# RomanBresson/KAGNN

Hardware: AMD Instinct MI355X
Metric: edges/sec KAN-GIN fwd+bwd, hidden=64 grid=5, 1M-node synthetic; HBM % peak (higher is better)
Workload: dtype f32 (fp16 hi/lo split operands, fp32 accumulate)

## Files before the change

### kagnn_amd/csrc/kan_split_bwd.hip

```cpp
#include <type_traits>
#include "split_common.h"

namespace kagnn {

int kan_dw_reduce(const float* slab, long NS, long per_slab, float* gcat, hipStream_t st);

int kan_dw_unpack(const float* gcat, int in, int out, int C, long inP, long outP, const float* sw,
                  const float* sc, float* g_bw, float* g_sw, float* g_sc, hipStream_t st);


bool kan_split_dx_ok(int in, int out, int G, int K) { return K >= 0 && K <= 4 && G + K <= 16; }
static inline int vshift(int C) { return C > 8 ? 1 : 0; }

static size_t dx_blk_bytes(int inv , int ob) {
    return kHdrBytes + (size_t)cdiv(inv, 16) * kCTmax * dx_q2(ob) * 2 * 1024;
}
bool kan_dx_w2_ok(int in, int out, int C, int K) { return K == 3 && C > 8 && C <= 16 && out <= kOutBlk; }
static int dx_inv(int in, int out, int C, int K) { return kan_dx_w2_ok(in, out, C, K) ? 32 * cdiv(in, 16) : (in << vshift(C)); }

size_t kan_split_pack_dx_bytes(int in, int out, int C, int K) {
    return (size_t)cdiv(out, kOutBlk) * dx_blk_bytes(dx_inv(in, out, C, K), min(out, kOutBlk));
}

__global__ void split_pack_dx_kernel(const float* __restrict__ bw, const float* __restrict__ sw,
                                     const float* __restrict__ sc, int in, int out, int C, int Q2,
                                     unsigned char* __restrict__ pack, int self_scale, int w2) {
    unsigned* hdr = reinterpret_cast<unsigned*>(pack);
    __shared__ float s_m[17];
    const float wmax = self_scale == 2 ? header_absmax(pack) : self_scale ? block_absmax_w(bw, sw, sc, in, out, C, s_m) : __uint_as_float(hdr[2]);
    const int e = scale_exp_from_max(wmax);
    const float wscale = ldexpf(1.0f, -e);
    if (blockIdx.x == 0 && threadIdx.x == 0) {
        reinterpret_cast<float*>(pack)[0] = ldexpf(1.0f, e - 10);
        reinterpret_cast<int*>(pack)[1] = e;
    }
    pack_dx_items(bw, sw, sc, in, out, C, Q2, pack, wscale, blockIdx.x * (long)blockDim.x + threadIdx.x, (long)gridDim.x * blockDim.x, w2);
}

int kan_split_pack_dx_noscale(const float* bw, const float* sw, const float* sc, int in, int out, int C, int K,
                              void* pack_dx, hipStream_t st) {
    const int w2 = kan_dx_w2_ok(in, out, C, K) ? 1 : 0;
    const int inv = dx_inv(in, out, C, K);
    const size_t stride = dx_blk_bytes(inv, min(out, kOutBlk));
    for (int b = 0; b * kOutBlk < out; ++b) {
        const int ob = min(kOutBlk, out - b * kOutBlk), Q2 = dx_q2(ob);
        const long o0 = (long)b * kOutBlk;
        const long items = (long)cdiv(inv, 16) * kCTmax * Q2 * 64;
        const bool two = (long)in * ob * C >= kAbsmaxTwoLaunchMin;
        unsigned char* pd = static_cast<unsigned char*>(pack_dx) + b * stride;
        if (two) { int rc = launch_absmax_partials(bw ? bw + o0 * in : nullptr, sw + o0 * in * C, sc ? sc + o0 * in : nullptr, in, ob, C, pd, st); if (rc) return rc; }
        split_pack_dx_kernel<<<(int)min((items + 1023) / 1024, two ? 256L : 64L), 1024, 0, st>>>(
            bw ? bw + o0 * in : nullptr, sw + o0 * in * C, sc ? sc + o0 * in : nullptr, in, ob, C, Q2, pd, two ? 2 : 1, w2);
        KAGNN_LAUNCH_CHECK();
    }
    return KAGNN_OK;
}

template <int K>
__device__ __forceinline__ float barrel_dot(const float (&d)[8], int m, const float (&dN)[K + 1]) {
    const int a = m >> 2, b = m & 3;
    float U[K + 4];
#pragma unroll
    for (int j = 0; j < K + 4; ++j) {
        float v = 0.0f;
#pragma unroll
        for (int aa = 0; aa < 4; ++aa) {
            const int c = 4 * aa + j - K;
            if (c >= 0 && c < 8) v = (a == aa) ? d[c] : v;
        }
        U[j] = v;
    }
    float s = 0.0f;
#pragma unroll
    for (int r = 0; r <= K; ++r) {
        float e = U[r];
#pragma unroll
        for (int bb = 1; bb < 4; ++bb) e = (b == bb) ? U[r + bb] : e;
        s = fmaf(e, dN[r], s);
    }
    return s;
}


template <int K, int Q2, bool GEN, int PP, bool GX16 = false, bool BNB = false, bool XAFF = false, bool XST = false, bool HALF = false>
__global__ __launch_bounds__(512) void kan_split_dx_kernel(
    const float* __restrict__ x, long ldx, const float* __restrict__ gy, long ldgy, long N, int in,
    int out, int C, const float* __restrict__ knots_g, int nknots,
    const unsigned char* __restrict__ pack, int resident, float* __restrict__ gx, long ldgx,
    RbfArgs rb, int sh_arg , int acc_arg,
    int ft_per_block , BnBack bnb) {
    static_assert(!BNB || (K == 3 && !GEN && PP == 0 && !GX16), "the fused normalisation backward serves the lean cubic instantiation");
    static_assert(!XAFF || (K == 3 && !GEN && !GX16 && !BNB), "the input affine serves the lean cubic instantiation (the read-out of the node models)");
    static_assert(!XST || XAFF, "the column statistics ride in the read-out instantiation");
    static_assert(!HALF || (K == 3 && !GEN), "single-product mode: the lean cubic instantiation");
    const int sh = GEN ? sh_arg : 0;
    const bool ACC = GEN && acc_arg;
    extern __shared__ __attribute__((aligned(16))) unsigned char smem[];
    float* s_knots = reinterpret_cast<float*>(smem);
    unsigned char* s_w = smem + kLdsHdr;
    const int tid = threadIdx.x, wave = tid >> 6, lane = tid & 63;
    if (K > 0 && tid < nknots) s_knots[tid] = knots_g[tid];
    unsigned* s_btbl = reinterpret_cast<unsigned*>(smem + 256);
    constexpr unsigned gxes = GX16 ? 2u : 4u;
    if (K == 3) build_barrel_table(s_btbl, tid);
    const int inv = in << sh, FT = cdiv(inv, 16);
    constexpr int FT_BYTES = kCTmax * Q2 * 2 * 1024;
    const int e_w = reinterpret_cast<const int*>(pack)[1];
    const unsigned char* gw = pack + kHdrBytes;
    const unsigned lds_w = (unsigned)(size_t)((__attribute__((address_space(3))) unsigned char*)s_w);
    auto stage = [&](int ft0, int nft) {
        const unsigned char* src = gw + (size_t)ft0 * FT_BYTES;
        const int nblk = nft * (FT_BYTES / 1024);
        if constexpr (HALF) {
            for (int blk = 2 * wave; blk < nblk; blk += 16)
                lds_dma_1k(src + (size_t)blk * 1024 + lane * 16, __builtin_amdgcn_readfirstlane(lds_w + blk * 1024));
        } else
        for (int blk = wave; blk < nblk; blk += 8)
            lds_dma_1k(src + (size_t)blk * 1024 + lane * 16, __builtin_amdgcn_readfirstlane(lds_w + blk * 1024));
        lds_dma_wait();
    };
    const int ft_begin = blockIdx.y * ft_per_block, ft_end = min(FT, ft_begin + ft_per_block);
    if (resident) stage(ft_begin, ft_end - ft_begin);
    __syncthreads();
    const bool pingpong = (PP == 2) && resident;
    SplineGeom geom{}; FastGeom fgeo{};
    const int li = lane & 15, kg = lane >> 4;
    const int win = li & sh;
    float ca[8] = {};
    if constexpr (K == 0) {
        float c0[8], c1[8];
        rbf_centers(rb, c0, 0); rbf_centers(rb, c1, sh);
#pragma unroll
        for (int g = 0; g < 8; ++g) ca[g] = win ? c1[g] : c0[g];
    }
    if constexpr (K > 0) { geom = geom_from_knots(s_knots, nknots); fgeo = fast_geom(s_knots, nknots); }
    const bool ln_on = (K == 0) && rb.ln_w != nullptr;
    const bool al4 = ((ldgy & 3) == 0) && ((reinterpret_cast<uintptr_t>(gy) & 15) == 0);
    const unsigned ldx4 = (unsigned)ldx * 4u, ldgy4 = (unsigned)ldgy * 4u, ldgx4 = (unsigned)ldgx * gxes;
    const unsigned gy_ro = (unsigned)(wave * 32 + li) * ldgy4;
    const unsigned x_rb = (unsigned)(wave * 32 + 4 * kg) * ldx4;
    const unsigned gx_rb = (unsigned)(wave * 32 + 4 * kg) * ldgx4;
    const unsigned gz_rb = (unsigned)(wave * 32 + 4 * kg) * (unsigned)in * 4u;

    auto load_gy = [&](long tile, float (&raw)[2][Q2][8]) {
        const GBuf gyb = gbuf_at(gy, N, ldgy, out, tile * 256);
#pragma unroll
        for (int rt = 0; rt < 2; ++rt) {
            const unsigned ro = gy_ro + kg * 32;
            const unsigned so = (unsigned)(16 * rt) * ldgy4;
#pragma unroll
            for (int q = 0; q < Q2; ++q) {
                if (al4 && 32 * Q2 == out) {
                    gld4_s(gyb, ro, so + 128 * q, raw[rt][q]);
                    gld4_s(gyb, ro, so + 128 * q + 16, raw[rt][q] + 4);
                } else if (al4 && (out & 7) == 0) {
                    const unsigned rq = gy_ro + (unsigned)min(32 * q + 8 * kg, out - 8) * 4u;
                    gld4_s(gyb, rq, so, raw[rt][q]);
                    gld4_s(gyb, rq, so + 16, raw[rt][q] + 4);
                } else {
                    const int o0 = 32 * q + 8 * kg;
#pragma unroll
                    for (int j = 0; j < 8; ++j) raw[rt][q][j] = gld_s(gyb, gy_ro + min(o0 + j, out - 1) * 4, so);
                }
            }
        }
        if constexpr (BNB) {
            const GBuf yb = gbuf_at(bnb.y, N, bnb.ldy, out, tile * 256), ob = gbuf_at(bnb.gy_out, N, bnb.ldo, out, tile * 256);
            const unsigned ldy4 = (unsigned)bnb.ldy * 4u, ldo4 = (unsigned)bnb.ldo * 4u;
            const unsigned yro = (unsigned)(wave * 32 + li) * ldy4 + kg * 32, oro = (unsigned)(wave * 32 + li) * ldo4 + kg * 32;
#pragma unroll
            for (int q = 0; q < Q2; ++q) {
                float cm[8], cA[8], cB[8], cC[8];
                const float* t0 = bnb.tab + 32 * q + 8 * kg;
#pragma unroll
                for (int h = 0; h < 2; ++h) {
                    const float4 a = *reinterpret_cast<const float4*>(t0 + 4 * h), b = *reinterpret_cast<const float4*>(t0 + bnb.ldt + 4 * h);
                    const float4 c = *reinterpret_cast<const float4*>(t0 + 2 * bnb.ldt + 4 * h), d = *reinterpret_cast<const float4*>(t0 + 3 * bnb.ldt + 4 * h);
                    cm[4 * h] = a.x; cm[4 * h + 1] = a.y; cm[4 * h + 2] = a.z; cm[4 * h + 3] = a.w;
                    cA[4 * h] = b.x; cA[4 * h + 1] = b.y; cA[4 * h + 2] = b.z; cA[4 * h + 3] = b.w;
                    cB[4 * h] = c.x; cB[4 * h + 1] = c.y; cB[4 * h + 2] = c.z; cB[4 * h + 3] = c.w;
                    cC[4 * h] = d.x; cC[4 * h + 1] = d.y; cC[4 * h + 2] = d.z; cC[4 * h + 3] = d.w;
                }
#pragma unroll
                for (int rt = 0; rt < 2; ++rt) {
                    float yv[8];
                    gld4_s(yb, yro, (unsigned)(16 * rt) * ldy4 + 128 * q, yv);
                    gld4_s(yb, yro, (unsigned)(16 * rt) * ldy4 + 128 * q + 16, yv + 4);
#pragma unroll
                    for (int j = 0; j < 8; ++j) raw[rt][q][j] = bn_bwd_value(raw[rt][q][j], yv[j], cm[j], cA[j], cB[j], cC[j]);
                    if (blockIdx.y == 0) {
                        gst4_s(ob, oro, (unsigned)(16 * rt) * ldo4 + 128 * q, raw[rt][q]);
                        gst4_s(ob, oro, (unsigned)(16 * rt) * ldo4 + 128 * q + 16, raw[rt][q] + 4);
                    }
                }
            }
        }
    };
    u32x4 ahi[2][Q2], alo[2][Q2];
    float rinv[2][4];
    auto split_gy = [&](const float (&raw)[2][Q2][8]) {
#pragma unroll
        for (int rt = 0; rt < 2; ++rt) {
            float mx = 0.0f;
#pragma unroll
            for (int q = 0; q < Q2; ++q)
#pragma unroll
                for (int j = 0; j < 8; ++j) mx = fmaxf(mx, fabsf(raw[rt][q][j]));
            mx = fmaxf(mx, __shfl_xor(mx, 16));
            mx = fmaxf(mx, __shfl_xor(mx, 32));
            const int rexp = exp_for_max(mx);
            const float sc = ldexpf(1.0f, 10 - rexp);
#pragma unroll
            for (int q = 0; q < Q2; ++q) {
                float v[8];
#pragma unroll
                for (int j = 0; j < 8; ++j) v[j] = raw[rt][q][j] * sc;
                if constexpr (HALF) round_f16x2(v, ahi[rt][q]);
                else split_f16x2_asm(v, ahi[rt][q], alo[rt][q]);
            }
            const float mine = ldexpf(1.0f, e_w + rexp - 10);
#pragma unroll
            for (int reg = 0; reg < 4; ++reg) rinv[rt][reg] = __shfl(mine, 4 * kg + reg);
        }
    };
    float mu[2][4], rs[2][4];
    auto load_stats = [&](long tile) {
        if (ln_on) {
            const long row0 = tile * 256 + wave * 32;
#pragma unroll
            for (int rt = 0; rt < 2; ++rt)
#pragma unroll
                for (int reg = 0; reg < 4; ++reg) {
                    const long rc = min(row0 + 16 * rt + 4 * kg + reg, N - 1);
                    mu[rt][reg] = rb.stats[2 * rc]; rs[rt][reg] = rb.stats[2 * rc + 1];
                }
        }
    };

    float* s_stat = reinterpret_cast<float*>(s_w + (size_t)(ft_end - ft_begin) * FT_BYTES) + wave * 128;
    if constexpr (XST) { s_stat[lane] = 0.0f; s_stat[64 + lane] = 0.0f; }
    float graw[2][Q2][8];
    long tile = blockIdx.x;
    if (!XST && tile * 256 >= N) return;
    if (!XST || tile * 256 < N) {
    load_gy(tile, graw);
    load_stats(tile);
    split_gy(graw);
    if (PP >= 1 && (tile + gridDim.x) * 256 < N) load_gy(tile + gridDim.x, graw);
    }
    if (pingpong && wave >= 4) __builtin_amdgcn_s_barrier();

    for (; tile * 256 < N; tile += gridDim.x) {
        const bool more = (tile + gridDim.x) * 256 < N;
        if (PP == 0 && tile != (long)blockIdx.x) {
            load_gy(tile, graw);
            load_stats(tile);
            split_gy(graw);
        }
        const GBuf gzb = gbuf_at(rb.gz, N, in, in, tile * 256);
        const GBuf xb = gbuf_at(x, N, ldx, in, tile * 256), gxb = gbuf_at_es(gx, N, ldgx, in, tile * 256, (int)gxes);

        for (int ft = ft_begin; ft < ft_end; ++ft) {
            if (!resident) {
                __syncthreads();
                stage(ft, 1);
                __syncthreads();
            }
            const unsigned char* wft = s_w + (size_t)(resident ? ft - ft_begin : 0) * FT_BYTES + lane * 16;
            const int f = 16 * ft + li;
            const int fr = f >> sh;
            const unsigned fcol = (unsigned)min(fr, in - 1) * 4u;
            const unsigned gx_ro = gx_rb + (unsigned)min(fr, in - 1) * gxes, gz_ro = gz_rb + fcol;
            float gam = 1.0f, bet = 0.0f;
            if (ln_on) { gam = rb.ln_w[min(fr, in - 1)]; bet = rb.ln_b[min(fr, in - 1)]; }
            float xa = 1.0f, xs = 0.0f;
            if constexpr (XAFF) { xa = rb.x_affine[min(fr, in - 1)]; xs = rb.x_affine[in + min(fr, in - 1)]; }
            float st_m = 0.0f, st_q = 0.0f, st_g = 0.0f, st_gx = 0.0f;
            if constexpr (XST) { st_m = rb.st_mean[min(fr, in - 1)]; st_q = rb.st_rstd[min(fr, in - 1)]; }
            float xq[2][4];
#pragma unroll
            for (int rt = 0; rt < 2; ++rt)
#pragma unroll
                for (int reg = 0; reg < 4; ++reg) {
                    xq[rt][reg] = gld_s(xb, x_rb + fcol, (unsigned)(16 * rt + reg) * ldx4);
                }
            f32x4 D[kCTmax][2];
#pragma unroll
            for (int c = 0; c < kCTmax; ++c) { D[c][0] = f32x4{0.f, 0.f, 0.f, 0.f}; D[c][1] = f32x4{0.f, 0.f, 0.f, 0.f}; }
            {
                constexpr int NGRP = kCTmax * Q2;
#ifndef KAGNN_DX_LDS_DEPTH
#define KAGNN_DX_LDS_DEPTH 1
#endif
                constexpr int RD = KAGNN_DX_LDS_DEPTH;
                u32x4 bh[RD + 1], bl[RD + 1];
#pragma unroll
                for (int g = 0; g < RD; ++g) {
                    bh[g] = *reinterpret_cast<const u32x4*>(wft + (size_t)(2 * g + 0) * 1024);
                    if constexpr (!HALF) bl[g] = *reinterpret_cast<const u32x4*>(wft + (size_t)(2 * g + 1) * 1024);
                }
#pragma unroll
                for (int g = 0; g < NGRP; ++g) {
                    const int c = g / Q2, q = g % Q2;
                    if (g + RD < NGRP) {
                        bh[(g + RD) % (RD + 1)] = *reinterpret_cast<const u32x4*>(wft + (size_t)(2 * (g + RD) + 0) * 1024);
                        if constexpr (!HALF) bl[(g + RD) % (RD + 1)] = *reinterpret_cast<const u32x4*>(wft + (size_t)(2 * (g + RD) + 1) * 1024);
                    }
                    __builtin_amdgcn_sched_barrier(0);
                    const u32x4 bhi = bh[g % (RD + 1)];
                    D[c][0] = mfma16_f16(ahi[0][q], bhi, D[c][0]);
                    D[c][1] = mfma16_f16(ahi[1][q], bhi, D[c][1]);
                    if constexpr (!HALF) {
                        const u32x4 blo = bl[g % (RD + 1)];
                        D[c][0] = mfma16_f16(ahi[0][q], blo, D[c][0]);
                        D[c][1] = mfma16_f16(ahi[1][q], blo, D[c][1]);
                        D[c][0] = mfma16_f16(alo[0][q], bhi, D[c][0]);
                        D[c][1] = mfma16_f16(alo[1][q], bhi, D[c][1]);
                    }
                    __builtin_amdgcn_sched_barrier(0);
                }
            }
            if (pingpong) __builtin_amdgcn_s_barrier();
#pragma unroll
            for (int rt = 0; rt < 2; ++rt) {
#pragma unroll
                for (int reg = 0; reg < 4; ++reg) {
                    const float xv = XAFF ? fmaf(xq[rt][reg], xa, xs) : xq[rt][reg];
                    if constexpr (K == 0) {
                        const float z = ln_on ? fmaf((xv - mu[rt][reg]) * rs[rt][reg], gam, bet) : xv;
                        const float t0 = z * rb.a;
                        float sgz = 0.0f;
#pragma unroll
                        for (int g = 0; g < kCTmax - 1; ++g) {
                            const float t = t0 - ca[g];
                            sgz = fmaf(D[g][rt][reg], __builtin_amdgcn_exp2f(-t * t) * t, sgz);
                        }
                        float vz = sgz * rb.k2 * rinv[rt][reg];
                        float vb = D[kCTmax - 1][rt][reg] * silu_gradf(xv) * rinv[rt][reg];
                        if (sh) vz += __shfl_xor(vz, 1);
                        const unsigned so_x = (unsigned)(16 * rt + reg) * ldgx4, so_z = (unsigned)(16 * rt + reg) * (unsigned)in * 4u;
                        if (f < inv && win == 0) {
                            if (ln_on) {
                                if (ACC) { vz += gld_s(gzb, gz_ro, so_z); vb += gld_s(gxb, gx_ro, so_x); }
                                gst_s(gzb, gz_ro, so_z, vz);
                                gst_s(gxb, gx_ro, so_x, vb);
                            } else {
                                float v = vz + vb;
                                if (ACC) v += gld_s(gxb, gx_ro, so_x);
                                gst_s(gxb, gx_ro, so_x, v);
                            }
                        }
                    } else {
                    float dN[K + 1];
                    int m;
                    if constexpr (K == 3) {
#ifdef KAGNN_ABLATE_SHARED_EXPANSION
                        m = (int)(__float_as_uint(xv) & 7u);
                        dN[0] = xv; dN[1] = xv; dN[2] = xv; dN[3] = xv;
#else
                        const float t = fmaf(xv, fgeo.inv_h, fgeo.c0);
                        const float u = __builtin_amdgcn_fractf(t);
                        m = (int)floorf(t);
                        cubic_dbases(u, 1.0f, dN);
#endif
                    } else {
                        float Nv[K + 1];
                        m = bspline_local<K, true>(xv, s_knots, geom, Nv, dN);
                    }
                    float d[kCTmax - 1];
#pragma unroll
                    for (int c = 0; c < kCTmax - 1; ++c) d[c] = D[c][rt][reg];
                    float bar;
                    if constexpr (K == 3) {
                        const int mm = m - 8 * win;
                        const unsigned* be = s_btbl + kBarrelDw * min((unsigned)mm, 15u);
                        const u32x4 sel = *reinterpret_cast<const u32x4*>(be);
                        const uint2 rot = *reinterpret_cast<const uint2*>(be + 4);
                        bar = barrel_dot3(d, sel, rot.x, rot.y, dN) * (0.5f * fgeo.inv_h);
                    } else {
                        bar = barrel_dot<K>(d, m - 8 * win, dN);
                    }
                    float s = fmaf(D[kCTmax - 1][rt][reg], silu_gradf(xv), bar) * rinv[rt][reg];
                    if (sh) s += __shfl_xor(s, 1);
                    if constexpr (XST) {
                        st_g += s;
                        st_gx = fmaf(s, (xq[rt][reg] - st_m) * st_q, st_gx);
                    }
                    if (f < inv && win == 0) {
                        const unsigned so_x = (unsigned)(16 * rt + reg) * ldgx4;
                        if (ACC) s += gld_s(gxb, gx_ro, so_x);
                        if constexpr (GX16) gst16_s(gxb, gx_ro, so_x, s);
                        else gst_s(gxb, gx_ro, so_x, s);
                    }
                    }
                }
            }
            if constexpr (XST) {
                st_g += __shfl_xor(st_g, 16); st_gx += __shfl_xor(st_gx, 16);
                st_g += __shfl_xor(st_g, 32); st_gx += __shfl_xor(st_gx, 32);
                if (kg == 0 && f < in) { s_stat[f] += st_g; s_stat[64 + f] += st_gx; }
            }
            if (PP >= 1 && ft + 1 == ft_end && more) {
                load_stats(tile + gridDim.x);
                split_gy(graw);
                if ((tile + 2 * (long)gridDim.x) * 256 < N) load_gy(tile + 2 * (long)gridDim.x, graw);
            }
            if (pingpong) __builtin_amdgcn_s_barrier();
        }
    }
    if (pingpong && wave < 4) __builtin_amdgcn_s_barrier();
    if constexpr (XST) {
        __syncthreads();
        if (tid < 128) {
            const float* base = reinterpret_cast<const float*>(s_w + (size_t)(ft_end - ft_begin) * FT_BYTES);
            float a = 0.0f;
#pragma unroll
            for (int w8 = 0; w8 < 8; ++w8) a += base[w8 * 128 + tid];
            const int stat = tid >> 6, col = tid & 63;
            if (col < in) rb.st_partial[((long)blockIdx.x * 2 + stat) * in + col] = a;
        }
    }
}

template <int K, int Q2, bool GEN, int PP, bool GX16 = false, bool BNB = false, bool XAFF = false, bool XST = false, bool HALF = false>
static int launch_dx_pp(const float* x, long ldx, const float* gy, long ldgy, long N, int in, int out, int C,
                        const float* knots, int nknots, const unsigned char* pack, float* gx, long ldgx,
                        const RbfArgs& rb, int accumulate, hipStream_t st, const BnBack& bnb = BnBack{}) {
    if constexpr (!HALF && K == 3 && !GEN && Q2 <= 2 && PP != 2) {
        if (g_half_products)
            return launch_dx_pp<K, Q2, GEN, PP, GX16, BNB, XAFF, XST, true>(x, ldx, gy, ldgy, N, in, out, C, knots, nknots, pack, gx, ldgx, rb, accumulate, st, bnb);
    }
    const int sh = vshift(C), FT = cdiv(in << sh, 16);
    const size_t ft_bytes = (size_t)kCTmax * Q2 * 2 * 1024;
    const size_t budget = 160 * 1024 - kLdsHdr;
    const long row_blocks = cdiv(N, 256);
    int splits = row_blocks >= 128 ? 1 : (int)min((long)FT, 256 / row_blocks);
    const int fpb = cdiv(FT, splits);
    splits = cdiv(FT, fpb);
    const bool resident = (size_t)fpb * ft_bytes <= budget;
    if (XST && !(resident && splits == 1 && in <= 64 && (size_t)fpb * ft_bytes + 8 * 128 * sizeof(float) <= budget))
        return fail(KAGNN_ERR_UNSUPPORTED, "%s: column statistics need <= 64 input features, resident weights and >= 32768 rows", "kan_split_dx");
    const size_t lds = kLdsHdr + (resident ? fpb : 1) * ft_bytes + (XST ? 8 * 128 * sizeof(float) : 0);
    static unsigned long long configured = 0;
    if (auto first_use_ = first_use_on_this_device(configured)) {
        KAGNN_HIP(hipFuncSetAttribute((const void*)kan_split_dx_kernel<K, Q2, GEN, PP, GX16, BNB, XAFF, XST, HALF>,
                                      hipFuncAttributeMaxDynamicSharedMemorySize, (int)(160 * 1024)));
    }
    const dim3 grid((unsigned)min(row_blocks, 256L), (unsigned)splits);
    kan_split_dx_kernel<K, Q2, GEN, PP, GX16, BNB, XAFF, XST, HALF><<<grid, 512, lds, st>>>(x, ldx, gy, ldgy, N, in, out, C, knots, nknots, pack,
                                                                           resident ? 1 : 0, gx, ldgx, rb, sh, accumulate, fpb, bnb);
    KAGNN_LAUNCH_CHECK();
    return KAGNN_OK;
}

template <int K, int Q2, bool GEN>
static int launch_dx(const float* x, long ldx, const float* gy, long ldgy, long N, int in, int out, int C,
                     const float* knots, int nknots, const unsigned char* pack, float* gx, long ldgx,
                     const RbfArgs& rb, int accumulate, int gx16, hipStream_t st) {
    if constexpr (K == 3 && !GEN && Q2 == 4) {
        if (gx16) return launch_dx_pp<K, Q2, GEN, 0, true>(x, ldx, gy, ldgy, N, in, out, C, knots, nknots, pack, gx, ldgx, rb, accumulate, st);
        return launch_dx_pp<K, Q2, GEN, 0>(x, ldx, gy, ldgy, N, in, out, C, knots, nknots, pack, gx, ldgx, rb, accumulate, st);
    } else if constexpr (K == 3 && !GEN) {
        if (rb.x_affine) {
            if (gx16) return fail(KAGNN_ERR_UNSUPPORTED, "%s: an input affine and bf16 gradient rows do not combine", "kan_split_dx");
            if (rb.st_partial) {
                if constexpr (Q2 <= 2)
                    return launch_dx_pp<K, Q2, GEN, 1, false, false, true, true>(x, ldx, gy, ldgy, N, in, out, C, knots, nknots, pack, gx, ldgx, rb, accumulate, st);
                return fail(KAGNN_ERR_UNSUPPORTED, "%s: column statistics need <= 64 outputs", "kan_split_dx");
            }
            return launch_dx_pp<K, Q2, GEN, 1, false, false, true>(x, ldx, gy, ldgy, N, in, out, C, knots, nknots, pack, gx, ldgx, rb, accumulate, st);
        }
        if (gx16) return launch_dx_pp<K, Q2, GEN, 1, true>(x, ldx, gy, ldgy, N, in, out, C, knots, nknots, pack, gx, ldgx, rb, accumulate, st);
        return launch_dx_pp<K, Q2, GEN, 1>(x, ldx, gy, ldgy, N, in, out, C, knots, nknots, pack, gx, ldgx, rb, accumulate, st);
    }
    if (gx16) return fail(KAGNN_ERR_UNSUPPORTED, "%s: bf16 gradient rows need a cubic layer with <= 8 coefficients", "kan_split_dx");
    if (rb.x_affine) return fail(KAGNN_ERR_UNSUPPORTED, "%s: an input affine needs a cubic layer with <= 8 coefficients and <= 64 outputs", "kan_split_dx");
    return launch_dx_pp<K, Q2, GEN, 0>(x, ldx, gy, ldgy, N, in, out, C, knots, nknots, pack, gx, ldgx, rb, accumulate, st);
}

template <int Q2, int NS1>
__global__ __launch_bounds__(512) void kan_split_dx_w2_kernel(
    const float* __restrict__ x, long ldx, const float* __restrict__ gy, long ldgy, long N, int in, int out, int C,
    const float* __restrict__ knots_g, int nknots, const unsigned char* __restrict__ pack,
    float* __restrict__ gx, long ldgx) {
    extern __shared__ __attribute__((aligned(16))) unsigned char smem[];
    float* s_knots = reinterpret_cast<float*>(smem);
    unsigned* s_btbl = reinterpret_cast<unsigned*>(smem + 256);
    unsigned char* s_w = smem + kLdsHdr;
    const int tid = threadIdx.x, wave = tid >> 6, lane = tid & 63;
    if (tid < nknots) s_knots[tid] = knots_g[tid];
    build_barrel_table(s_btbl, tid);
    const int T = cdiv(in, 16);
    constexpr int ns1 = NS1;
    constexpr int FT_BYTES = kCTmax * Q2 * 2 * 1024;
    const int e_w = reinterpret_cast<const int*>(pack)[1];
    const unsigned char* gw = pack + kHdrBytes;
    const unsigned lds_w = (unsigned)(size_t)((__attribute__((address_space(3))) unsigned char*)s_w);
    auto stage_issue = [&](int tile, int nslots, unsigned dst_off) {
        const unsigned char* src = gw + (size_t)tile * FT_BYTES;
        const int nblk = nslots * Q2 * 2;
        for (int blk = wave; blk < nblk; blk += 8)
            lds_dma_1k(src + blk * 1024 + lane * 16, __builtin_amdgcn_readfirstlane(lds_w + dst_off + blk * 1024));
    };
    constexpr bool AHEAD = !(Q2 == 4 && NS1 == 4);
    __syncthreads();
    if (AHEAD && (long)blockIdx.x * 256 < N) stage_issue(0, kCTmax, 0u);
    const FastGeom fgeo = fast_geom(s_knots, nknots);
    const float wd = 0.5f * fgeo.inv_h;
    const int li = lane & 15, kg = lane >> 4;
    const bool al4 = ((ldgy & 3) == 0) && ((reinterpret_cast<uintptr_t>(gy) & 15) == 0) && (32 * Q2 == out);
    const unsigned ldx4 = (unsigned)ldx * 4u, ldgy4 = (unsigned)ldgy * 4u, ldgx4 = (unsigned)ldgx * 4u;
    const unsigned gy_ro = (unsigned)(wave * 32 + li) * ldgy4;
    const unsigned x_rb = (unsigned)(wave * 32 + 4 * kg) * ldx4;
    const unsigned gx_rb = (unsigned)(wave * 32 + 4 * kg) * ldgx4;
    const unsigned char* wl = s_w + lane * 16;
    const unsigned char* wl1 = wl + FT_BYTES;

    for (long tile = blockIdx.x; tile * 256 < N; tile += gridDim.x) {
        const GBuf gyb = gbuf_at(gy, N, ldgy, out, tile * 256);
        const GBuf xb = gbuf_at(x, N, ldx, in, tile * 256), gxb = gbuf_at(gx, N, ldgx, in, tile * 256);
        u32x4 ahi[2][Q2], alo[2][Q2];
        float rinv[2][4];
#pragma unroll
        for (int rt = 0; rt < 2; ++rt) {
            const unsigned ro = gy_ro + kg * 32, so = (unsigned)(16 * rt) * ldgy4;
            float raw[Q2][8];
            float mx = 0.0f;
#pragma unroll
            for (int q = 0; q < Q2; ++q) {
                if (al4) {
                    gld4_s(gyb, ro, so + 128 * q, raw[q]);
                    gld4_s(gyb, ro, so + 128 * q + 16, raw[q] + 4);
                } else {
                    const int o0 = 32 * q + 8 * kg;
#pragma unroll
                    for (int j = 0; j < 8; ++j) raw[q][j] = gld_s(gyb, gy_ro + min(o0 + j, out - 1) * 4, so);
                }
#pragma unroll
                for (int j = 0; j < 8; ++j) mx = fmaxf(mx, fabsf(raw[q][j]));
            }
            mx = fmaxf(mx, __shfl_xor(mx, 16));
            mx = fmaxf(mx, __shfl_xor(mx, 32));
            const int rexp = exp_for_max(mx);
            const float sc = ldexpf(1.0f, 10 - rexp);
#pragma unroll
            for (int q = 0; q < Q2; ++q) {
                float v[8];
#pragma unroll
                for (int j = 0; j < 8; ++j) v[j] = raw[q][j] * sc;
                split_f16x2_asm(v, ahi[rt][q], alo[rt][q]);
            }
            const float mine = ldexpf(1.0f, e_w + rexp - 10);
#pragma unroll
            for (int reg = 0; reg < 4; ++reg) rinv[rt][reg] = __shfl(mine, 4 * kg + reg);
        }

        for (int t = 0; t < T; ++t) {
            const int f = 16 * t + li;
            const unsigned fcol = (unsigned)min(f, in - 1) * 4u;
            float xq[2][4];
#pragma unroll
            for (int rt = 0; rt < 2; ++rt)
#pragma unroll
                for (int reg = 0; reg < 4; ++reg) xq[rt][reg] = gld_s(xb, x_rb + fcol, (unsigned)(16 * rt + reg) * ldx4);
            f32x4 D[kCTmax][2];
            if constexpr (AHEAD) {
                lds_dma_wait();
                __syncthreads();
            } else {
                __syncthreads();
                stage_issue(2 * t, kCTmax, 0u); lds_dma_wait();
                __syncthreads();
            }
#pragma unroll
            for (int c = 0; c < kCTmax; ++c) { D[c][0] = f32x4{0.f, 0.f, 0.f, 0.f}; D[c][1] = f32x4{0.f, 0.f, 0.f, 0.f}; }
            {
                constexpr int NGRP = kCTmax * Q2;
                u32x4 bh[2], bl[2];
                bh[0] = *reinterpret_cast<const u32x4*>(wl + 0 * 1024);
                bl[0] = *reinterpret_cast<const u32x4*>(wl + 1 * 1024);
#pragma unroll
                for (int g = 0; g < NGRP; ++g) {
                    const int c = g / Q2, q = g % Q2;
                    if (g + 1 < NGRP) {
                        bh[(g + 1) & 1] = *reinterpret_cast<const u32x4*>(wl + (size_t)(2 * (g + 1) + 0) * 1024);
                        bl[(g + 1) & 1] = *reinterpret_cast<const u32x4*>(wl + (size_t)(2 * (g + 1) + 1) * 1024);
                    }
                    __builtin_amdgcn_sched_barrier(0);
                    const u32x4 bhi = bh[g & 1], blo = bl[g & 1];
                    D[c][0] = mfma16_f16(ahi[0][q], bhi, D[c][0]);
                    D[c][1] = mfma16_f16(ahi[1][q], bhi, D[c][1]);
                    D[c][0] = mfma16_f16(ahi[0][q], blo, D[c][0]);
                    D[c][1] = mfma16_f16(ahi[1][q], blo, D[c][1]);
                    D[c][0] = mfma16_f16(alo[0][q], bhi, D[c][0]);
                    D[c][1] = mfma16_f16(alo[1][q], bhi, D[c][1]);
                    __builtin_amdgcn_sched_barrier(0);
                }
            }
            float s0[2][4];
#pragma unroll
            for (int rt = 0; rt < 2; ++rt) {
                __builtin_amdgcn_sched_barrier(0);
#pragma unroll
                for (int reg = 0; reg < 4; ++reg) {
                    const float xv = xq[rt][reg];
                    const float tt = fmaf(xv, fgeo.inv_h, fgeo.c0);
                    const float u = __builtin_amdgcn_fractf(tt);
                    const int m = (int)floorf(tt);
                    float dN[4];
                    cubic_dbases(u, 1.0f, dN);
                    float d[kCTmax - 1];
#pragma unroll
                    for (int c = 0; c < kCTmax - 1; ++c) d[c] = D[c][rt][reg];
                    const unsigned* be = s_btbl + kBarrelDw * min((unsigned)m, 15u);
                    const u32x4 sel = *reinterpret_cast<const u32x4*>(be);
                    const uint2 rot = *reinterpret_cast<const uint2*>(be + 4);
                    s0[rt][reg] = fmaf(D[kCTmax - 1][rt][reg], silu_gradf(xv), barrel_dot3(d, sel, rot.x, rot.y, dN) * wd);
                }
            }
            __syncthreads();
            stage_issue(2 * t + 1, ns1, (unsigned)FT_BYTES); lds_dma_wait();
            __syncthreads();
            if constexpr (AHEAD) {
                if (t + 1 < T) stage_issue(2 * (t + 1), kCTmax, 0u);
                else if ((tile + gridDim.x) * 256 < N) stage_issue(0, kCTmax, 0u);
            }
            f32x4 D1[NS1][2];
#pragma unroll
            for (int c = 0; c < NS1; ++c) { D1[c][0] = f32x4{0.f, 0.f, 0.f, 0.f}; D1[c][1] = f32x4{0.f, 0.f, 0.f, 0.f}; }
#pragma unroll
            for (int c = 0; c < NS1; ++c) {
#pragma unroll
                for (int q = 0; q < Q2; ++q) {
                    const u32x4 bhi = *reinterpret_cast<const u32x4*>(wl1 + (size_t)(2 * (c * Q2 + q) + 0) * 1024);
                    const u32x4 blo = *reinterpret_cast<const u32x4*>(wl1 + (size_t)(2 * (c * Q2 + q) + 1) * 1024);
                    D1[c][0] = mfma16_f16(ahi[0][q], bhi, D1[c][0]);
                    D1[c][1] = mfma16_f16(ahi[1][q], bhi, D1[c][1]);
                    D1[c][0] = mfma16_f16(ahi[0][q], blo, D1[c][0]);
                    D1[c][1] = mfma16_f16(ahi[1][q], blo, D1[c][1]);
                    D1[c][0] = mfma16_f16(alo[0][q], bhi, D1[c][0]);
                    D1[c][1] = mfma16_f16(alo[1][q], bhi, D1[c][1]);
                    __builtin_amdgcn_sched_barrier(0);
                }
            }
            const unsigned gx_ro = gx_rb + fcol;
#pragma unroll
            for (int rt = 0; rt < 2; ++rt) {
                __builtin_amdgcn_sched_barrier(0);
#pragma unroll
                for (int reg = 0; reg < 4; ++reg) {
                    const float tt = fmaf(xq[rt][reg], fgeo.inv_h, fgeo.c0);
                    const float u = __builtin_amdgcn_fractf(tt);
                    const int m = (int)floorf(tt);
                    float dN[4];
                    cubic_dbases(u, 1.0f, dN);
                    float d[kCTmax - 1];
#pragma unroll
                    for (int c = 0; c < kCTmax - 1; ++c) d[c] = c < NS1 ? D1[c < NS1 ? c : 0][rt][reg] : 0.0f;
                    const int m1 = m - 8;
                    const unsigned* be = s_btbl + kBarrelDw * min((unsigned)m1, 15u);
                    const u32x4 sel = *reinterpret_cast<const u32x4*>(be);
                    const uint2 rot = *reinterpret_cast<const uint2*>(be + 4);
                    const float s = fmaf(barrel_dot3(d, sel, rot.x, rot.y, dN), wd, s0[rt][reg]) * rinv[rt][reg];
                    if (f < in) gst_s(gxb, gx_ro, (unsigned)(16 * rt + reg) * ldgx4, s);
                }
            }
        }
    }
}

template <int Q2, int NS1>
static int launch_dx_w2(const float* x, long ldx, const float* gy, long ldgy, long N, int in, int out, int C,
                        const float* knots, int nknots, const unsigned char* pack, float* gx, long ldgx, hipStream_t st) {
    const size_t lds = kLdsHdr + (size_t)(kCTmax + NS1) * Q2 * 2 * 1024;
    static unsigned long long configured = 0;
    if (auto first_use_ = first_use_on_this_device(configured)) {
        KAGNN_HIP(hipFuncSetAttribute((const void*)kan_split_dx_w2_kernel<Q2, NS1>, hipFuncAttributeMaxDynamicSharedMemorySize, (int)(160 * 1024)));
    }
    kan_split_dx_w2_kernel<Q2, NS1><<<(unsigned)min((long)cdiv(N, 256), 256L), 512, lds, st>>>(x, ldx, gy, ldgy, N, in, out, C, knots, nknots,
                                                                                        pack, gx, ldgx);
    KAGNN_LAUNCH_CHECK();
    return KAGNN_OK;
}

static int dx_block(const float* x, long ldx, const float* gy, long ldgy, long N, const float* knots, int in,
                    int out, int G, int K, const unsigned char* p, float* gx, long ldgx, const RbfArgs& rb,
                    int accumulate, int gx16, hipStream_t st) {
    const int C = G + K, nk = K ? G + 2 * K + 1 : 0, Q2 = dx_q2(out);
#define GO(KK, QQ) return (accumulate || C > 8) ? launch_dx<KK, QQ, true>(x, ldx, gy, ldgy, N, in, out, C, knots, nk, p, gx, ldgx, rb, accumulate, gx16, st) \
                                                 : launch_dx<KK, QQ, false>(x, ldx, gy, ldgy, N, in, out, C, knots, nk, p, gx, ldgx, rb, 0, gx16, st)
#define BYQ(KK) switch (Q2) { case 1: GO(KK, 1); case 2: GO(KK, 2); case 4: GO(KK, 4); }
    switch (K) {
        case 0: BYQ(0) break;
        case 1: BYQ(1) break;
        case 2: BYQ(2) break;
        case 3: BYQ(3) break;
        case 4: BYQ(4) break;
    }
#undef BYQ
#undef GO
    return fail(KAGNN_ERR_UNSUPPORTED, "%s: shape not covered by the split path", "kan_split_dx");
}

int kan_split_dx_any(const float* x, long ldx, const float* gy, long ldgy, long N, const float* knots, int in,
                     int out, int G, int K, const void* pack, float* gx, long ldgx, const RbfArgs& rb,
                     hipStream_t st, int gx16) {
    if (gx16 && (K == 0 || out > kOutBlk))
        return fail(KAGNN_ERR_UNSUPPORTED, "%s: bf16 gradient rows need a B-spline layer with <= 128 outputs", "kan_split_dx");
    if (kan_dx_w2_ok(in, out, G + K, K)) {
        if (gx16) return fail(KAGNN_ERR_UNSUPPORTED, "%s: bf16 gradient rows need <= 8 coefficients", "kan_split_dx");
        const unsigned char* p = static_cast<const unsigned char*>(pack);
        const int nk = G + 2 * K + 1;
#define W2Q(QQ, NN) launch_dx_w2<QQ, NN>(x, ldx, gy, ldgy, N, in, out, G + K, knots, nk, p, gx, ldgx, st)
#define W2(QQ) switch (G + K - 8) { case 1: return W2Q(QQ, 1); case 2: return W2Q(QQ, 2); case 3: return W2Q(QQ, 3); case 4: return W2Q(QQ, 4); \
                                    default: return W2Q(QQ, 8); }
        switch (dx_q2(out)) {
            case 1: W2(1)
            case 2: W2(2)
            default:
                switch (G + K - 8) { case 1: case 2: return W2Q(4, 2); case 3: return W2Q(4, 3); case 4: return W2Q(4, 4); default: return W2Q(4, 8); }
        }
#undef W2
#undef W2Q
    }
    const size_t stride = dx_blk_bytes(in << vshift(G + K), min(out, kOutBlk));
    for (int b = 0; b * kOutBlk < out; ++b) {
        const int rc = dx_block(x, ldx, gy + b * kOutBlk, ldgy, N, knots, in, min(kOutBlk, out - b * kOutBlk), G, K,
                                static_cast<const unsigned char*>(pack) + b * stride, gx, ldgx, rb, b > 0, gx16, st);
        if (rc) return rc;
    }
    return KAGNN_OK;
}

bool kan_split_dx_bn_ok(long ldg, int in, int out, int G, int K, const BnBack& b, const void* g) {
    auto al = [](const void* p) { return (reinterpret_cast<uintptr_t>(p) & 15) == 0; };
    return K == 3 && G + K <= 8 && (out == 32 || out == 64) && !kan_dx_w2_ok(in, out, G + K, K) && ldg % 4 == 0 && b.ldy % 4 == 0 &&
           b.ldo % 4 == 0 && b.ldt % 4 == 0 && b.ldt >= out && b.ldy <= 7680 && b.ldo <= 7680 && al(g) && al(b.y) && al(b.gy_out) && al(b.tab);
}
int kan_split_dx_bn(const float* x, long ldx, const float* g, long ldg, long N, const float* knots, int in, int out, int G, int K,
                    const void* pack, float* gx, long ldgx, const BnBack& bnb, hipStream_t st) {
    if (!kan_split_dx_bn_ok(ldg, in, out, G, K, bnb, g)) return fail(KAGNN_ERR_UNSUPPORTED, "%s: shape not covered", "kan_split_dx_bn");
    const unsigned char* p = static_cast<const unsigned char*>(pack);
    const int nk = G + 2 * K + 1;
    if (out == 32) return launch_dx_pp<3, 1, false, 0, false, true>(x, ldx, g, ldg, N, in, out, G + K, knots, nk, p, gx, ldgx, RbfArgs{}, 0, st, bnb);
    return launch_dx_pp<3, 2, false, 0, false, true>(x, ldx, g, ldg, N, in, out, G + K, knots, nk, p, gx, ldgx, RbfArgs{}, 0, st, bnb);
}

int kan_split_dx_stats_blocks(long N) { return (int)min((long)cdiv(N, 256), 256L); }
bool kan_split_dx_stats_ok(long N, int in, int out, int G, int K) {
    return K == 3 && G + K <= 8 && in <= 64 && in % 4 == 0 && out <= 64 && cdiv(N, 256) >= 128;
}
int kan_split_dx_stats(const float* x, long ldx, const float* gy, long ldgy, long N, const float* knots, int in, int out, int G, int K,
                       const void* pack, float* gx, long ldgx, hipStream_t st, const float* x_affine, const float* st_mean,
// ... 968 lines not shown
```

Measured before the change: 4.329 billion.

## Add transposed-accumulator dx kernel for vectorized x loads and gx stores

Adds a TR variant of the cubic split dx kernel that swaps the MFMA operand order, so each lane holds four consecutive input features of one row instead of four rows of one feature. x is then read and gx written with 16-byte vector accesses per row rather than scalar strided accesses, and the per-row scale shuffle is dropped. The launcher uses it when in is a multiple of 16 and pointers and strides are aligned. It also adds compile-time ablation macros that disable the path. Risks are correctness across the wave layout and a changed per-feature affine gather.

```diff
diff --git a/kagnn_amd/csrc/kan_split_bwd.hip b/kagnn_amd/csrc/kan_split_bwd.hip
--- a/kagnn_amd/csrc/kan_split_bwd.hip
+++ b/kagnn_amd/csrc/kan_split_bwd.hip
@@ -8,6 +8,15 @@
 int kan_dw_unpack(const float* gcat, int in, int out, int C, long inP, long outP, const float* sw,
                   const float* sc, float* g_bw, float* g_sw, float* g_sc, hipStream_t st);
 
+
+#if defined(KAGNN_ABLATE_DX_XGX) || defined(KAGNN_ABLATE_DX_SEL) || defined(KAGNN_ABLATE_DX_LEAN)
+#define KAGNN_DX_ROW_GROUPS 1
+#endif
+#ifdef KAGNN_DX_ROW_GROUPS
+constexpr bool kDxRowGroups = true;
+#else
+constexpr bool kDxRowGroups = false;
+#endif
 
 bool kan_split_dx_ok(int in, int out, int G, int K) { return K >= 0 && K <= 4 && G + K <= 16; }
 static inline int vshift(int C) { return C > 8 ? 1 : 0; }
@@ -82,17 +91,18 @@
 }
 
 
-template <int K, int Q2, bool GEN, int PP, bool GX16 = false, bool BNB = false, bool XAFF = false, bool XST = false, bool HALF = false>
-__global__ __launch_bounds__(512) void kan_split_dx_kernel(
+template <int K, int Q2, bool GEN, int PP, bool GX16, bool BNB, bool XAFF, bool XST, bool HALF, bool TR>
+__device__ __forceinline__ void kan_split_dx_body(
     const float* __restrict__ x, long ldx, const float* __restrict__ gy, long ldgy, long N, int in,
     int out, int C, const float* __restrict__ knots_g, int nknots,
     const unsigned char* __restrict__ pack, int resident, float* __restrict__ gx, long ldgx,
-    RbfArgs rb, int sh_arg , int acc_arg,
-    int ft_per_block , BnBack bnb) {
+    const RbfArgs& rb, int sh_arg , int acc_arg,
+    int ft_per_block , const BnBack& bnb) {
     static_assert(!BNB || (K == 3 && !GEN && PP == 0 && !GX16), "the fused normalisation backward serves the lean cubic instantiation");
     static_assert(!XAFF || (K == 3 && !GEN && !GX16 && !BNB), "the input affine serves the lean cubic instantiation (the read-out of the node models)");
     static_assert(!XST || XAFF, "the column statistics ride in the read-out instantiation");
     static_assert(!HALF || (K == 3 && !GEN), "single-product mode: the lean cubic instantiation");
+    static_assert(!TR || (K == 3 && !GEN && !GX16 && !XST), "the transposed accumulator serves the lean cubic instantiation with fp32 rows");
     const int sh = GEN ? sh_arg : 0;
     const bool ACC = GEN && acc_arg;
     extern __shared__ __attribute__((aligned(16))) unsigned char smem[];
@@ -123,6 +133,10 @@
     if (resident) stage(ft_begin, ft_end - ft_begin);
     __syncthreads();
     const bool pingpong = (PP == 2) && resident;
+#ifdef KAGNN_ABLATE_DX_SEL
+    const u32x4 abl_sel = *reinterpret_cast<const u32x4*>(s_btbl + kBarrelDw * 5);
+    const uint2 abl_rot = *reinterpret_cast<const uint2*>(s_btbl + kBarrelDw * 5 + 4);
+#endif
     SplineGeom geom{}; FastGeom fgeo{};
     const int li = lane & 15, kg = lane >> 4;
     const int win = li & sh;
@@ -141,6 +155,8 @@
     const unsigned x_rb = (unsigned)(wave * 32 + 4 * kg) * ldx4;
     const unsigned gx_rb = (unsigned)(wave * 32 + 4 * kg) * ldgx4;
     const unsigned gz_rb = (unsigned)(wave * 32 + 4 * kg) * (unsigned)in * 4u;
+    const unsigned x_tr = (unsigned)(wave * 32 + li) * ldx4 + kg * 16;
+    const unsigned gx_tr = (unsigned)(wave * 32 + li) * ldgx4 + kg * 16;
 
     auto load_gy = [&](long tile, float (&raw)[2][Q2][8]) {
         const GBuf gyb = gbuf_at(gy, N, ldgy, out, tile * 256);
@@ -220,7 +236,7 @@
             }
             const float mine = ldexpf(1.0f, e_w + rexp - 10);
 #pragma unroll
-            for (int reg = 0; reg < 4; ++reg) rinv[rt][reg] = __shfl(mine, 4 * kg + reg);
+            for (int reg = 0; reg < 4; ++reg) rinv[rt][reg] = TR ? mine : __shfl(mine, 4 * kg + reg);
         }
     };
     float mu[2][4], rs[2][4];
@@ -269,24 +285,50 @@
             const unsigned char* wft = s_w + (size_t)(resident ? ft - ft_begin : 0) * FT_BYTES + lane * 16;
             const int f = 16 * ft + li;
             const int fr = f >> sh;
+#ifdef KAGNN_ABLATE_DX_LEAN
+            const unsigned fcol = (unsigned)fr * 4u;
+            const unsigned gx_ro = gx_rb + (unsigned)fr * gxes, gz_ro = gz_rb + fcol;
+#else
             const unsigned fcol = (unsigned)min(fr, in - 1) * 4u;
             const unsigned gx_ro = gx_rb + (unsigned)min(fr, in - 1) * gxes, gz_ro = gz_rb + fcol;
+#endif
             float gam = 1.0f, bet = 0.0f;
             if (ln_on) { gam = rb.ln_w[min(fr, in - 1)]; bet = rb.ln_b[min(fr, in - 1)]; }
-            float xa = 1.0f, xs = 0.0f;
-            if constexpr (XAFF) { xa = rb.x_affine[min(fr, in - 1)]; xs = rb.x_affine[in + min(fr, in - 1)]; }
+            float xa[4] = {1.0f, 1.0f, 1.0f, 1.0f}, xs[4] = {};
+            if constexpr (XAFF) {
+#pragma unroll
+                for (int reg = 0; reg < 4; ++reg) {
+                    const int fa = TR ? 16 * ft + 4 * kg + reg : min(fr, in - 1);
+                    xa[reg] = rb.x_affine[fa]; xs[reg] = rb.x_affine[in + fa];
+                }
+            }
             float st_m = 0.0f, st_q = 0.0f, st_g = 0.0f, st_gx = 0.0f;
             if constexpr (XST) { st_m = rb.st_mean[min(fr, in - 1)]; st_q = rb.st_rstd[min(fr, in - 1)]; }
             float xq[2][4];
+#ifdef KAGNN_ABLATE_DX_XGX
+            float abl_sum = 0.0f;
+#pragma unroll
+            for (int rt = 0; rt < 2; ++rt)
+#pragma unroll
+                for (int reg = 0; reg < 4; ++reg) xq[rt][reg] = (float)(lane + 8 * rt + reg) * 0.01f - 0.5f;
+#else
+            if constexpr (TR) {
+#pragma unroll
+                for (int rt = 0; rt < 2; ++rt) gld4_s(xb, x_tr, (unsigned)(16 * rt) * ldx4 + 64u * (unsigned)ft, xq[rt]);
+            } else
 #pragma unroll
             for (int rt = 0; rt < 2; ++rt)
 #pragma unroll
                 for (int reg = 0; reg < 4; ++reg) {
                     xq[rt][reg] = gld_s(xb, x_rb + fcol, (unsigned)(16 * rt + reg) * ldx4);
                 }
+#endif
             f32x4 D[kCTmax][2];
 #pragma unroll
             for (int c = 0; c < kCTmax; ++c) { D[c][0] = f32x4{0.f, 0.f, 0.f, 0.f}; D[c][1] = f32x4{0.f, 0.f, 0.f, 0.f}; }
+            auto mm = [](const u32x4& g_frag, const u32x4& w_frag, const f32x4& acc) {
+                return TR ? mfma16_f16(w_frag, g_frag, acc) : mfma16_f16(g_frag, w_frag, acc);
+            };
             {
                 constexpr int NGRP = kCTmax * Q2;
 #ifndef KAGNN_DX_LDS_DEPTH
@@ -308,14 +350,14 @@
                     }
                     __builtin_amdgcn_sched_barrier(0);
                     const u32x4 bhi = bh[g % (RD + 1)];
-                    D[c][0] = mfma16_f16(ahi[0][q], bhi, D[c][0]);
-                    D[c][1] = mfma16_f16(ahi[1][q], bhi, D[c][1]);
+                    D[c][0] = mm(ahi[0][q], bhi, D[c][0]);
+                    D[c][1] = mm(ahi[1][q], bhi, D[c][1]);
                     if constexpr (!HALF) {
                         const u32x4 blo = bl[g % (RD + 1)];
-                        D[c][0] = mfma16_f16(ahi[0][q], blo, D[c][0]);
-                        D[c][1] = mfma16_f16(ahi[1][q], blo, D[c][1]);
-                        D[c][0] = mfma16_f16(alo[0][q], bhi, D[c][0]);
-                        D[c][1] = mfma16_f16(alo[1][q], bhi, D[c][1]);
+                        D[c][0] = mm(ahi[0][q], blo, D[c][0]);
+                        D[c][1] = mm(ahi[1][q], blo, D[c][1]);
+                        D[c][0] = mm(alo[0][q], bhi, D[c][0]);
+                        D[c][1] = mm(alo[1][q], bhi, D[c][1]);
                     }
                     __builtin_amdgcn_sched_barrier(0);
                 }
@@ -325,7 +367,7 @@
             for (int rt = 0; rt < 2; ++rt) {
 #pragma unroll
                 for (int reg = 0; reg < 4; ++reg) {
-                    const float xv = XAFF ? fmaf(xq[rt][reg], xa, xs) : xq[rt][reg];
+                    const float xv = XAFF ? fmaf(xq[rt][reg], xa[reg], xs[reg]) : xq[rt][reg];
                     if constexpr (K == 0) {
                         const float z = ln_on ? fmaf((xv - mu[rt][reg]) * rs[rt][reg], gam, bet) : xv;
                         const float t0 = z * rb.a;
@@ -372,10 +414,15 @@
                     for (int c = 0; c < kCTmax - 1; ++c) d[c] = D[c][rt][reg];
                     float bar;
                     if constexpr (K == 3) {
-                        const int mm = m - 8 * win;
-                        const unsigned* be = s_btbl + kBarrelDw * min((unsigned)mm, 15u);
+                        const int mw = m - 8 * win;
+#ifdef KAGNN_ABLATE_DX_SEL
+                        const u32x4 sel = abl_sel; const uint2 rot = abl_rot;
+                        dN[0] += __int_as_float(mw & 1);
+#else
+                        const unsigned* be = s_btbl + kBarrelDw * min((unsigned)mw, 15u);
                         const u32x4 sel = *reinterpret_cast<const u32x4*>(be);
                         const uint2 rot = *reinterpret_cast<const uint2*>(be + 4);
+#endif
                         bar = barrel_dot3(d, sel, rot.x, rot.y, dN) * (0.5f * fgeo.inv_h);
                     } else {
                         bar = barrel_dot<K>(d, m - 8 * win, dN);
@@ -386,15 +433,30 @@
                         st_g += s;
                         st_gx = fmaf(s, (xq[rt][reg] - st_m) * st_q, st_gx);
                     }
+#ifdef KAGNN_ABLATE_DX_XGX
+                    abl_sum += s;
+#else
+                    if constexpr (TR) {
+                        xq[rt][reg] = s;
+                    } else
+#ifdef KAGNN_ABLATE_DX_LEAN
+                    if (true) {
+#else
                     if (f < inv && win == 0) {
+#endif
                         const unsigned so_x = (unsigned)(16 * rt + reg) * ldgx4;
                         if (ACC) s += gld_s(gxb, gx_ro, so_x);
                         if constexpr (GX16) gst16_s(gxb, gx_ro, so_x, s);
                         else gst_s(gxb, gx_ro, so_x, s);
                     }
+#endif
                     }
                 }
-            }
+                if constexpr (TR) gst4_s(gxb, gx_tr, (unsigned)(16 * rt) * ldgx4 + 64u * (unsigned)ft, xq[rt]);
+            }
+#ifdef KAGNN_ABLATE_DX_XGX
+            gst_s(gxb, gx_ro, 0u, abl_sum);
+#endif
             if constexpr (XST) {
                 st_g += __shfl_xor(st_g, 16); st_gx += __shfl_xor(st_gx, 16);
                 st_g += __shfl_xor(st_g, 32); st_gx += __shfl_xor(st_gx, 32);
@@ -423,12 +485,34 @@
 }
 
 template <int K, int Q2, bool GEN, int PP, bool GX16 = false, bool BNB = false, bool XAFF = false, bool XST = false, bool HALF = false>
+__global__ __launch_bounds__(512) void kan_split_dx_kernel(
+    const float* __restrict__ x, long ldx, const float* __restrict__ gy, long ldgy, long N, int in, int out, int C,
+    const float* __restrict__ knots_g, int nknots, const unsigned char* __restrict__ pack, int resident, float* __restrict__ gx, long ldgx,
+    RbfArgs rb, int sh_arg, int acc_arg, int ft_per_block, BnBack bnb) {
+    kan_split_dx_body<K, Q2, GEN, PP, GX16, BNB, XAFF, XST, HALF, false>(x, ldx, gy, ldgy, N, in, out, C, knots_g, nknots, pack, resident, gx, ldgx,
+                                                                          rb, sh_arg, acc_arg, ft_per_block, bnb);
+}
+template <int K, int Q2, bool GEN, int PP, bool GX16 = false, bool BNB = false, bool XAFF = false, bool XST = false, bool HALF = false>
+__global__ __launch_bounds__(512) void kan_split_dx_tr_kernel(
+    const float* __restrict__ x, long ldx, const float* __restrict__ gy, long ldgy, long N, int in, int out, int C,
+    const float* __restrict__ knots_g, int nknots, const unsigned char* __restrict__ pack, int resident, float* __restrict__ gx, long ldgx,
+    RbfArgs rb, int sh_arg, int acc_arg, int ft_per_block, BnBack bnb) {
+    kan_split_dx_body<K, Q2, GEN, PP, GX16, BNB, XAFF, XST, HALF, true>(x, ldx, gy, ldgy, N, in, out, C, knots_g, nknots, pack, resident, gx, ldgx,
+                                                                         rb, sh_arg, acc_arg, ft_per_block, bnb);
+}
+
+template <int K, int Q2, bool GEN, int PP, bool GX16 = false, bool BNB = false, bool XAFF = false, bool XST = false, bool HALF = false, bool TR = false>
 static int launch_dx_pp(const float* x, long ldx, const float* gy, long ldgy, long N, int in, int out, int C,
                         const float* knots, int nknots, const unsigned char* pack, float* gx, long ldgx,
                         const RbfArgs& rb, int accumulate, hipStream_t st, const BnBack& bnb = BnBack{}) {
     if constexpr (!HALF && K == 3 && !GEN && Q2 <= 2 && PP != 2) {
         if (g_half_products)
             return launch_dx_pp<K, Q2, GEN, PP, GX16, BNB, XAFF, XST, true>(x, ldx, gy, ldgy, N, in, out, C, knots, nknots, pack, gx, ldgx, rb, accumulate, st, bnb);
+    }
+    if constexpr (!TR && K == 3 && !GEN && !GX16 && !XST) {
+        auto al = [](const void* p) { return (reinterpret_cast<uintptr_t>(p) & 15) == 0; };
+        if (in % 16 == 0 && ldx % 4 == 0 && ldgx % 4 == 0 && al(x) && al(gx) && !kDxRowGroups)
+            return launch_dx_pp<K, Q2, GEN, PP, GX16, BNB, XAFF, XST, HALF, true>(x, ldx, gy, ldgy, N, in, out, C, knots, nknots, pack, gx, ldgx, rb, accumulate, st, bnb);
     }
     const int sh = vshift(C), FT = cdiv(in << sh, 16);
     const size_t ft_bytes = (size_t)kCTmax * Q2 * 2 * 1024;
@@ -441,14 +525,20 @@
     if (XST && !(resident && splits == 1 && in <= 64 && (size_t)fpb * ft_bytes + 8 * 128 * sizeof(float) <= budget))
         return fail(KAGNN_ERR_UNSUPPORTED, "%s: column statistics need <= 64 input features, resident weights and >= 32768 rows", "kan_split_dx");
     const size_t lds = kLdsHdr + (resident ? fpb : 1) * ft_bytes + (XST ? 8 * 128 * sizeof(float) : 0);
+    const void* kern;
+    if constexpr (TR) kern = (const void*)kan_split_dx_tr_kernel<K, Q2, GEN, PP, GX16, BNB, XAFF, XST, HALF>;
+    else kern = (const void*)kan_split_dx_kernel<K, Q2, GEN, PP, GX16, BNB, XAFF, XST, HALF>;
     static unsigned long long configured = 0;
     if (auto first_use_ = first_use_on_this_device(configured)) {
-        KAGNN_HIP(hipFuncSetAttribute((const void*)kan_split_dx_kernel<K, Q2, GEN, PP, GX16, BNB, XAFF, XST, HALF>,
-                                      hipFuncAttributeMaxDynamicSharedMemorySize, (int)(160 * 1024)));
+        KAGNN_HIP(hipFuncSetAttribute(kern, hipFuncAttributeMaxDynamicSharedMemorySize, (int)(160 * 1024)));
     }
     const dim3 grid((unsigned)min(row_blocks, 256L), (unsigned)splits);
-    kan_split_dx_kernel<K, Q2, GEN, PP, GX16, BNB, XAFF, XST, HALF><<<grid, 512, lds, st>>>(x, ldx, gy, ldgy, N, in, out, C, knots, nknots, pack,
-                                                                           resident ? 1 : 0, gx, ldgx, rb, sh, accumulate, fpb, bnb);
+    if constexpr (TR)
+        kan_split_dx_tr_kernel<K, Q2, GEN, PP, GX16, BNB, XAFF, XST, HALF><<<grid, 512, lds, st>>>(x, ldx, gy, ldgy, N, in, out, C, knots, nknots, pack,
+                                                                                  resident ? 1 : 0, gx, ldgx, rb, sh, accumulate, fpb, bnb);
+    else
+        kan_split_dx_kernel<K, Q2, GEN, PP, GX16, BNB, XAFF, XST, HALF><<<grid, 512, lds, st>>>(x, ldx, gy, ldgy, N, in, out, C, knots, nknots, pack,
+                                                                               resident ? 1 : 0, gx, ldgx, rb, sh, accumulate, fpb, bnb);
     KAGNN_LAUNCH_CHECK();
     return KAGNN_OK;
 }
```

Result: no change. 4.350 billion, median of 3 (+0.5%).
